# andrewcsmith/vox_box.rs

Hardware: AMD Instinct MI355X
Metric: frames/sec (pitch+LPC+formants), 48 kHz 25 ms/10 ms hop, 1→8 MI355X (higher is better)
Workload: dtype f64

## Files before the change

vox_box.rs_amd/csrc/vbx_device.hpp:

```cpp
#pragma once

#include <hip/hip_runtime.h>
#include <stdint.h>

#define VBX_WAVE 64

namespace vbx {


__device__ __forceinline__ double readlane_f64(double v, int lane) {
    int lo = __double2loint(v), hi = __double2hiint(v);
    lo = __builtin_amdgcn_readlane(lo, lane);
    hi = __builtin_amdgcn_readlane(hi, lane);
    return __hiloint2double(hi, lo);
}

__device__ __forceinline__ double readfirstlane_f64(double v) {
    int lo = __double2loint(v), hi = __double2hiint(v);
    lo = __builtin_amdgcn_readfirstlane(lo);
    hi = __builtin_amdgcn_readfirstlane(hi);
    return __hiloint2double(hi, lo);
}

template <int CTRL>
__device__ __forceinline__ double dpp_f64(double v) {
    int lo = __double2loint(v), hi = __double2hiint(v);
    lo = __builtin_amdgcn_update_dpp(0, lo, CTRL, 0xf, 0xf, true);
    hi = __builtin_amdgcn_update_dpp(0, hi, CTRL, 0xf, 0xf, true);
    return __hiloint2double(hi, lo);
}

constexpr int DPP_ROW_BCAST15 = 0x142, DPP_ROW_BCAST31 = 0x143;

constexpr int DPP_ROW_ROR1 = 0x121, DPP_ROW_ROR2 = 0x122, DPP_ROW_ROR4 = 0x124, DPP_ROW_ROR8 = 0x128;
constexpr int DPP_WAVE_SHL1 = 0x130;
constexpr int DPP_WAVE_SHR1 = 0x138;

__device__ __forceinline__ double from_next_lane(double v) { return dpp_f64<DPP_WAVE_SHL1>(v); }
__device__ __forceinline__ double from_prev_lane(double v) { return dpp_f64<DPP_WAVE_SHR1>(v); }

__device__ __forceinline__ double rounded(double v) { asm volatile("" : "+v"(v)); return v; }

__device__ __forceinline__ double wave_sum(double v) {
    v = rounded(v);
    v += dpp_f64<DPP_ROW_ROR8>(v);
    v += dpp_f64<DPP_ROW_ROR4>(v);
    v += dpp_f64<DPP_ROW_ROR2>(v);
    v += dpp_f64<DPP_ROW_ROR1>(v);
    double a = readlane_f64(v, 0), b = readlane_f64(v, 16), c = readlane_f64(v, 32), d = readlane_f64(v, 48);
    return (a + b) + (c + d);
}

template <int CTRL, int ROW_MASK>
__device__ __forceinline__ double dpp_f64_or_zero(double v) {
    int lo = __double2loint(v), hi = __double2hiint(v);
    lo = __builtin_amdgcn_update_dpp(0, lo, CTRL, ROW_MASK, 0xf, false);
    hi = __builtin_amdgcn_update_dpp(0, hi, CTRL, ROW_MASK, 0xf, false);
    return __hiloint2double(hi, lo);
}
__device__ __forceinline__ double wave_inclusive_scan(double v) {
    v += dpp_f64<0x111>(v);
    v += dpp_f64<0x112>(v);
    v += dpp_f64<0x114>(v);
    v += dpp_f64<0x118>(v);
    v += dpp_f64_or_zero<DPP_ROW_BCAST15, 0xA>(v);
    v += dpp_f64_or_zero<DPP_ROW_BCAST31, 0xC>(v);
    return v;
}

__device__ __forceinline__ double wave_max(double v) {
    v = fmax(v, dpp_f64<DPP_ROW_ROR8>(v));
    v = fmax(v, dpp_f64<DPP_ROW_ROR4>(v));
    v = fmax(v, dpp_f64<DPP_ROW_ROR2>(v));
    v = fmax(v, dpp_f64<DPP_ROW_ROR1>(v));
    double a = readlane_f64(v, 0), b = readlane_f64(v, 16), c = readlane_f64(v, 32), d = readlane_f64(v, 48);
    return fmax(fmax(a, b), fmax(c, d));
}

__device__ __forceinline__ double wave_sum_shfl(double v) {
    for (int o = 32; o > 0; o >>= 1) v += __shfl_xor(v, o, 64);
    return readfirstlane_f64(v);
}

__device__ __forceinline__ int lane_id() { return (int)(threadIdx.x & 63u); }

constexpr long XCD_RUN = 1024;
__device__ __forceinline__ long xcd_item(long b, long n) {
    constexpr long T = 8 * XCD_RUN;
    const long tile = b / T;
    if ((tile + 1) * T > n) return b;
    const long j = b - tile * T;
    return tile * T + (j & 7) * XCD_RUN + (j >> 3);
}

constexpr int DPP_QUAD_XOR1 = 0xB1;
constexpr int DPP_QUAD_REV = 0x1B;
constexpr int DPP_ROW_HALF_MIRROR = 0x141;
constexpr int DPP_ROW_MIRROR = 0x140;

template <int G>
__device__ __forceinline__ double group_sum(double v) {
    static_assert(G == 4 || G == 8 || G == 16 || G == 32 || G == 64, "group size");
    v = rounded(v);
    v += dpp_f64<DPP_QUAD_XOR1>(v);
    v += dpp_f64<DPP_QUAD_REV>(v);
    if (G >= 8) v += dpp_f64<DPP_ROW_HALF_MIRROR>(v);
    if (G >= 16) v += dpp_f64<DPP_ROW_MIRROR>(v);
    if (G == 64) {
        v += dpp_f64<DPP_ROW_BCAST15>(v);
        v += dpp_f64<DPP_ROW_BCAST31>(v);
        return readlane_f64(v, 63);
    }
    if (G == 32) {
        const double a = readlane_f64(v, 0), b = readlane_f64(v, 16), c = readlane_f64(v, 32), d = readlane_f64(v, 48);
        return (lane_id() < 32) ? (a + b) : (c + d);
    }
    return v;
}

__device__ __forceinline__ void wave_sync() {
    __builtin_amdgcn_fence(__ATOMIC_ACQ_REL, "wavefront");
    __builtin_amdgcn_wave_barrier();
}

__device__ __forceinline__ double rcp_nr1(double a) {
    double r = __builtin_amdgcn_rcp(a);
    return fma(fma(-a, r, 1.0), r, r);
}
__device__ __forceinline__ double rcp_nr2(double a) {
    double r = __builtin_amdgcn_rcp(a);
    r = fma(fma(-a, r, 1.0), r, r);
    return fma(fma(-a, r, 1.0), r, r);
}

__device__ __forceinline__ double div_exact_small(double x, double denom, double r) {
    const double q = x * r;
    const double rem = fma(-q, denom, x);
    return fma(rem, r, q);
}
__device__ __forceinline__ double pcm16_value(int s) { return div_exact_small((double)s, 32767.0, 1.0 / 32767.0); }


template <typename T> struct cx { T re, im; };
using c64 = cx<double>;
using c32 = cx<float>;

template <typename T> __device__ __forceinline__ cx<T> cmk(T re, T im) { cx<T> z; z.re = re; z.im = im; return z; }
template <typename T> __device__ __forceinline__ cx<T> cadd(cx<T> a, cx<T> b) { return cmk<T>(a.re + b.re, a.im + b.im); }
template <typename T> __device__ __forceinline__ cx<T> csub(cx<T> a, cx<T> b) { return cmk<T>(a.re - b.re, a.im - b.im); }
template <typename T> __device__ __forceinline__ cx<T> cneg(cx<T> a) { return cmk<T>(-a.re, -a.im); }
template <typename T> __device__ __forceinline__ cx<T> cmul(cx<T> a, cx<T> b) {
    return cmk<T>(a.re * b.re - a.im * b.im, a.re * b.im + a.im * b.re);
}
template <typename T> __device__ __forceinline__ cx<T> cmad(cx<T> a, cx<T> b, cx<T> c) {
    return cmk<T>(fma(a.re, b.re, fma(-a.im, b.im, c.re)), fma(a.re, b.im, fma(a.im, b.re, c.im)));
}
__device__ __forceinline__ double cdiv_recip(double ns) {
#ifdef VBX_IEEE_CDIV
    return 1.0 / ns;
#else
    return rcp_nr2(ns);
#endif
}
__device__ __forceinline__ float cdiv_recip(float ns) { return 1.0f / ns; }
template <typename T> __device__ __forceinline__ cx<T> cdiv(cx<T> a, cx<T> b) {
    T ns = b.re * b.re + b.im * b.im;
    T inv = cdiv_recip(ns);
    T re = a.re * b.re + a.im * b.im;
    T im = a.im * b.re - a.re * b.im;
    return cmk<T>(re * inv, im * inv);
}
template <typename T> __device__ __forceinline__ T cnorm(cx<T> a) { return hypot(a.re, a.im); }
template <typename T> __device__ __forceinline__ bool ciszero(cx<T> a) { return a.re == T(0) && a.im == T(0); }
template <typename T> __device__ __forceinline__ cx<T> csqrt(cx<T> z) {
    T r = hypot(z.re, z.im);
    if (r == T(0)) return cmk<T>(T(0), z.im);
    if (z.re >= T(0)) {
        T t = sqrt(T(0.5) * (r + z.re));
        return cmk<T>(t, z.im / (T(2) * t));
    }
    T t = sqrt(T(0.5) * (r - z.re));
    return cmk<T>(fabs(z.im) / (T(2) * t), copysign(t, z.im));
}

}
```

vox_box.rs_amd/csrc/vbx_pitch_refine.hpp:

```cpp
#pragma once
#include <type_traits>

#include "vbx_device.hpp"
#include "vbx_kernels.hpp"

namespace vbx {


__device__ __forceinline__ double fma_sc(double p, double x, const double c) {
    double r;
    asm("v_fma_f64 %0, %1, %2, %3" : "=v"(r) : "v"(p), "v"(x), "s"(c));
    return r;
}

__device__ __forceinline__ double sin_poly(double x) {
    const double x2 = x * x;
    double p = -1.9572941063391261231e-20;
    p = fma_sc(p, x2, 8.2206352466243297170e-18);
    p = fma_sc(p, x2, -2.8114572543455207632e-15);
    p = fma_sc(p, x2, 7.6471637318198164759e-13);
    p = fma_sc(p, x2, -1.6059043836821614599e-10);
    p = fma_sc(p, x2, 2.5052108385441718775e-08);
    p = fma_sc(p, x2, -2.7557319223985890653e-06);
    p = fma_sc(p, x2, 1.9841269841269841270e-04);
    p = fma_sc(p, x2, -8.3333333333333333333e-03);
    p = fma_sc(p, x2, 1.6666666666666666667e-01);
    return x * fma(-x2, p, 1.0);
}
__device__ __forceinline__ double cos_poly(double x) {
    const double x2 = x * x;
    double p = 8.8967913924505732867e-22;
    p = fma_sc(p, x2, -4.1103176233121648585e-19);
    p = fma_sc(p, x2, 1.5619206968586226462e-16);
    p = fma_sc(p, x2, -4.7794773323873852974e-14);
    p = fma_sc(p, x2, 1.1470745597729724714e-11);
    p = fma_sc(p, x2, -2.0876756987868098979e-09);
    p = fma_sc(p, x2, 2.7557319223985890653e-07);
    p = fma_sc(p, x2, -2.4801587301587301587e-05);
    p = fma_sc(p, x2, 1.3888888888888888889e-03);
    p = fma_sc(p, x2, -4.1666666666666666667e-02);
    p = fma(p, x2, 0.5);
    return fma(-x2, p, 1.0);
}

__device__ __forceinline__ double cos_0_pi(double theta) { return -sin_poly(theta - 1.57079632679489661923); }

__device__ __forceinline__ double y_at(const double *y, int nvalid, int idx) {
    return (idx < nvalid) ? y[idx] : 0.0;
}
__device__ __forceinline__ double y_at_padded(const double *y, int nvalid, int idx) {
    return y[(idx < nvalid) ? idx : nvalid - 1];
}


template <int G>
__device__ __forceinline__ double sinc_terms_general(const double *y, int nvalid, int ylen, int offset, int nl, int nr,
                                                     double phil, double phir, int max_depth, int lig = -1) {
    if (lig < 0) lig = lane_id() & (G - 1);
    const int side = lig & 1;
    const double ph = side ? phir : phil;
    const double s0 = sinpi(ph);
    const double inv_dd = 1.0 / (ph + (double)max_depth);
    const int ibase = side ? (offset + nl) : (offset + nr);
    double acc = 0.0;
    for (int n = (lig >> 1); n <= max_depth; n += G / 2) {
        const double a = M_PI * (ph + (double)n);
        int idx = side ? (ibase + n) : (ibase - n);
        idx = (idx < 0) ? 0 : idx;
        idx = (idx >= ylen) ? (ylen - 1) : idx;
        const double r_lag = y_at(y, nvalid, idx);
        const double sgn_s0 = (n & 1) ? -s0 : s0;
        const double first = sgn_s0 * rcp_nr2(a);
        const double second = fma(0.5, cos_0_pi(a * inv_dd), 0.5);
        acc = fma(r_lag * first, second, acc);
    }
    return acc;
}

struct sinc_stream_t {
    double pn, C, d, kappa, acc0, acc1;
    const double *yp;
};

template <int NSTEP>
__device__ __forceinline__ void sinc_stream_init(sinc_stream_t &s, const double *y, int side, int n0, int ibase_l, int ibase_r,
                                                 double phil, double phir, int max_depth) {
    constexpr double S = (double)NSTEP;
    const double ph = side ? phir : phil;
    const double h2 = M_PI * rcp_nr2(ph + (double)max_depth);
    s.pn = ph + (double)n0;
    const double theta0 = h2 * s.pn, delta = h2 * S;
    s.C = cos_0_pi(theta0);
    s.d = cos_0_pi(theta0 + delta) - s.C;
    const double sh = sin_poly(0.5 * delta);
    s.kappa = 4.0 * sh * sh;
    s.yp = y + (side ? (ibase_r + n0) : (ibase_l - n0));
    s.acc0 = 0.0; s.acc1 = 0.0;
}

template <int NSTEP>
__device__ __forceinline__ void sinc_stream_block4(sinc_stream_t &s, const int step) {
    constexpr double S = (double)NSTEP;
    const double y0 = s.yp[0], y1 = s.yp[step], y2 = s.yp[2 * step], y3 = s.yp[3 * step];
    const double p0 = s.pn, p1 = s.pn + S, p2 = s.pn + 2.0 * S, p3 = s.pn + 3.0 * S;
    const double q01 = p0 * p1, q23 = p2 * p3;
    const double r = rcp_nr1(q01 * q23);
    const double r01 = r * q23, r23 = r * q01;
    const double t0 = y0 * (r01 * p1), t1 = y1 * (r01 * p0), t2 = y2 * (r23 * p3), t3 = y3 * (r23 * p2);
    s.acc0 += t0; s.acc1 = fma(t0, s.C, s.acc1);
    s.C += s.d; s.d = fma(-s.kappa, s.C, s.d);
    s.acc0 += t1; s.acc1 = fma(t1, s.C, s.acc1);
    s.C += s.d; s.d = fma(-s.kappa, s.C, s.d);
    s.acc0 += t2; s.acc1 = fma(t2, s.C, s.acc1);
    s.C += s.d; s.d = fma(-s.kappa, s.C, s.d);
    s.acc0 += t3; s.acc1 = fma(t3, s.C, s.acc1);
    s.C += s.d; s.d = fma(-s.kappa, s.C, s.d);
    s.pn += 4.0 * S;
    s.yp += 4 * step;
}

template <int NSTEP>
__device__ __forceinline__ void sinc_stream_tail(sinc_stream_t &s, const int step, const int rem) {
    constexpr double S = (double)NSTEP;
    const double y0 = s.yp[0], y1 = (rem > 1) ? s.yp[step] : 0.0, y2 = (rem > 2) ? s.yp[2 * step] : 0.0;
    const double p0 = s.pn, p1 = s.pn + S, p2 = s.pn + 2.0 * S;
    const double q01 = p0 * p1;
    const double r = rcp_nr1(q01 * p2);
    const double r01 = r * p2;
    const double t0 = y0 * (r01 * p1), t1 = y1 * (r01 * p0), t2 = y2 * (r * q01);
    s.acc0 += t0; s.acc1 = fma(t0, s.C, s.acc1);
    s.C += s.d; s.d = fma(-s.kappa, s.C, s.d);
    s.acc0 += t1; s.acc1 = fma(t1, s.C, s.acc1);
    s.C += s.d;
    s.acc0 += t2; s.acc1 = fma(t2, s.C, s.acc1);
}

__device__ __forceinline__ double sinc_stream_result(const sinc_stream_t &s, int n0, double k) {
    const double acc = s.acc0 + s.acc1;
    return rounded(((n0 & 1) ? -acc : acc) * k);
}

template <int G>
__device__ __forceinline__ double sinc_terms_fast(const double *y, int ibase_l, int ibase_r,
                                                  double phil, double phir, int max_depth) {
    constexpr int NSTEP = G / 2;
    const int lig = lane_id() & (G - 1);
    const int side = lig & 1;
    const int n0 = lig >> 1;
    const double s0 = sin_poly(M_PI * fmin(phil, phir));
    const int nterms = (n0 <= max_depth) ? (max_depth - n0) / NSTEP + 1 : 0;
    sinc_stream_t s;
    sinc_stream_init<NSTEP>(s, y, side, n0, ibase_l, ibase_r, phil, phir, max_depth);
    const int step = side ? NSTEP : -NSTEP;
    int j = 0;
    for (; j + 4 <= nterms; j += 4) sinc_stream_block4<NSTEP>(s, step);
    if (j < nterms) sinc_stream_tail<NSTEP>(s, step, nterms - j);
    return sinc_stream_result(s, n0, s0 * (0.5 * 0.31830988618379067154));
}

__device__ __forceinline__ double sinc_terms_fast_cell(const double *yp0, int side, int n0, int nterms, double dmd,
                                                       double phil, double phir) {
    constexpr int NSTEP = 32;
    constexpr double S = (double)NSTEP;
    const int step = side ? NSTEP : -NSTEP;
    const double s0 = sin_poly(M_PI * fmin(phil, phir));
    sinc_stream_t s;
    const double ph = side ? phir : phil;
    const double h2 = M_PI * rcp_nr2(ph + dmd);
    s.pn = ph + (double)n0;
    const double theta0 = h2 * s.pn, delta = h2 * S;
    s.C = cos_0_pi(theta0);
    s.d = cos_0_pi(theta0 + delta) - s.C;
    const double sh = sin_poly(0.5 * delta);
    s.kappa = 4.0 * sh * sh;
    s.yp = yp0;
    s.acc0 = 0.0; s.acc1 = 0.0;
    int j = 0;
    for (; j + 4 <= nterms; j += 4) sinc_stream_block4<NSTEP>(s, step);
    if (j < nterms) sinc_stream_tail<NSTEP>(s, step, nterms - j);
    return sinc_stream_result(s, n0, s0 * (0.5 * 0.31830988618379067154));
}

template <int VG>
__device__ __forceinline__ double sinc_terms_fast_dual(const double *y, int ibase_l, int ibase_r,
                                                       double phil, double phir, int max_depth) {
    constexpr int NSTEP = VG / 2;
    const int n0 = lane_id() & (VG / 2 - 1);
    const double s0 = sin_poly(M_PI * fmin(phil, phir));
    const int nterms = (n0 <= max_depth) ? (max_depth - n0) / NSTEP + 1 : 0;
    sinc_stream_t sl, sr;
    sinc_stream_init<NSTEP>(sl, y, 0, n0, ibase_l, ibase_r, phil, phir, max_depth);
    sinc_stream_init<NSTEP>(sr, y, 1, n0, ibase_l, ibase_r, phil, phir, max_depth);
    int j = 0;
    for (; j + 4 <= nterms; j += 4) { sinc_stream_block4<NSTEP>(sl, -NSTEP); sinc_stream_block4<NSTEP>(sr, NSTEP); }
    if (j < nterms) { sinc_stream_tail<NSTEP>(sl, -NSTEP, nterms - j); sinc_stream_tail<NSTEP>(sr, NSTEP, nterms - j); }
    const double k = s0 * (0.5 * 0.31830988618379067154);
    return sinc_stream_result(sl, n0, k) + sinc_stream_result(sr, n0, k);
}

template <int G, bool DUAL = false>
__device__ __forceinline__ double sinc_interp(const double *y, int nvalid, int ylen, int offset, int nx,
                                              double x, int max_depth, bool active, int &st,
                                              unsigned *terms = nullptr, bool trusted = false) {
    bool summed = false, fast = false;
    double special = 0.0, phil = 0.5, phir = 0.5;
    int nl = 0, nr = 1;
    if (active && trusted) {
        const double fl = floor(x);
        nl = (int)fl;
        nr = nl + 1;
        phil = x - fl;
        phir = 1.0 - phil;
        if (fabs(x - (double)nl) < 1.0e-10) special = y[offset + nl];
        else if (fabs(x - (double)nr) < 1.0e-10) special = y[offset + nr];
        else {
            if ((offset + nr) < max_depth) max_depth = offset + nr;
            if ((offset + nl + max_depth) >= nx) max_depth = nx - offset + nl - 1;
            summed = true; fast = true;
        }
    } else if (active) {
        if (nx < 1) special = __builtin_nan("");
        else if (x > (double)nx) {
            const int idx = offset + nx - 1;
            if (idx < 0 || idx >= ylen) st |= 4; else special = y_at(y, nvalid, idx);
        } else if (x < 0.0) special = y_at(y, nvalid, 0);
        else {
            const double fl = floor(x);
            nl = (fl > 0.0) ? (int)fl : 0;
            nr = nl + 1;
            phil = x - (double)nl;
            phir = 1.0 - phil;
            if (fabs(x - (double)nl) < 1.0e-10) {
                const int idx = offset + nl;
                if (idx < 0 || idx >= ylen) st |= 4; else special = y_at(y, nvalid, idx);
            } else if (fabs(x - (double)nr) < 1.0e-10) {
                const int idx = offset + nr;
                if (idx < 0 || idx >= ylen) st |= 4; else special = y_at(y, nvalid, idx);
            } else {
                if ((offset + nr) < max_depth) max_depth = ((offset + nr) < 0) ? 0 : (offset + nr);
                if ((offset + nl + max_depth) >= nx) max_depth = nx - offset + nl - 1;
                if (max_depth < 0 || offset + nr >= ylen) st |= 4;
                else {
                    summed = true;
                    fast = !(x != x) && max_depth <= offset + nr && offset + nl >= 0 &&
                           offset + nl + max_depth < nvalid && offset + nr < nvalid;
                }
            }
        }
    }
    double acc = 0.0;
    if (terms != nullptr && summed) *terms += 2u * (unsigned)(max_depth + 1);
    if (summed) {
        if constexpr (DUAL) {
            if (fast) acc = sinc_terms_fast_dual<2 * G>(y, offset + nr, offset + nl, phil, phir, max_depth);
            else {
                const int p = lane_id() & (G - 1);
                acc = rounded(sinc_terms_general<2 * G>(y, nvalid, ylen, offset, nl, nr, phil, phir, max_depth, 2 * p)) +
                      rounded(sinc_terms_general<2 * G>(y, nvalid, ylen, offset, nl, nr, phil, phir, max_depth, 2 * p + 1));
            }
        } else {
            if (fast) acc = sinc_terms_fast<G>(y, offset + nr, offset + nl, phil, phir, max_depth);
            else acc = sinc_terms_general<G>(y, nvalid, ylen, offset, nl, nr, phil, phir, max_depth);
        }
    }
    const double total = group_sum<G>(acc);
    return summed ? total : special;
}

__device__ __forceinline__ bool sinc_bracket_trusted(double a0, double b0, int nvalid, int ylen, int offset, int nx, int depth) {
    if (!(a0 >= 0.0 && b0 <= (double)nx && b0 - a0 <= 2.5)) return false;
    const int lo = (int)floor(a0), hi = (int)floor(b0);
    bool ok = true;
    for (int nl = lo; nl <= hi; nl++) {
        const int nr = nl + 1;
        int D = depth;
        if ((offset + nr) < D) D = ((offset + nr) < 0) ? 0 : (offset + nr);
        if ((offset + nl + D) >= nx) D = nx - offset + nl - 1;
        ok = ok && D >= 0 && offset + nr < ylen && D <= offset + nr && offset + nl >= 0 && offset + nl + D < nvalid &&
             offset + nr < nvalid && offset + nr >= 1;
    }
    return ok;
}

template <int G>
__device__ __forceinline__ void improve_extremum_sinc(const double *y, int nvalid, int ylen, int offset, int nx,
                                                      double ixmid, int depth, bool active,
                                                      double &xmid, double &ymid, int &st,
                                                      unsigned *terms = nullptr, unsigned *evals = nullptr,
                                                      double bar = -__builtin_inf(), bool *pruned = nullptr,
                                                      bool negate = false ) {
#pragma clang fp contract(off)
    const double golden = 1. - 0.6180339887498948482045868343656381177203091798057628621;
    const double sqrt_epsilon = 1.4901161193847656e-08;
    const double eps = 2.220446049250313e-16;
    const double tol = 1e-10;
    xmid = 0.; ymid = 0.;
    bool run = active;
    if (active) {
        if (ixmid == 0.) { xmid = 0.; ymid = y_at(y, nvalid, 0); run = false; }
        else if (ixmid >= (double)nx) {
            run = false;
            if (nx < 1 || nx - 1 >= ylen) st |= 4;
            else { xmid = (double)nx; ymid = y_at(y, nvalid, nx - 1); }
        } else if (!(ixmid - 1. < ixmid + 1.)) { st |= 4; run = false; }
    }
    double a = ixmid - 1., b = ixmid + 1.;
    const bool trusted = run && sinc_bracket_trusted(a, b, nvalid, ylen, offset, nx, depth);
    double v = a + golden * (b - a);
    double fv = sinc_interp<G>(y, nvalid, ylen, offset, nx, v, depth, run, st, terms, trusted);
    if (negate) fv = -fv;
    if (evals != nullptr && run) *evals += 1u;
    double x = v, w = v, fx = fv, fw = fv;
    bool done = !run;
    const bool prunable = pruned != nullptr && run && a >= (double)(-offset);
    if (pruned != nullptr) {
        const double ub = (fv <= 1.) ? fv : 1.;
        *pruned = prunable && ub < bar;
        done = done || *pruned;
    }
    for (int it = 1; it <= 60; it++) {
        const double range = b - a;
        const double middle_range = (a + b) * 0.5;
        const double tol_act = sqrt_epsilon * fabs(x) + tol / 3.;
        if (!done && fabs(x - middle_range) + range * 0.5 <= 2. * tol_act) done = true;
        if (!__any(!done)) break;
        double new_step = (x < middle_range) ? golden * (b - x) : golden * (a - x);
        if (fabs(x - w) >= tol_act) {
            const double t = (x - w) * (fx - fv);
            double q = (x - v) * (fx - fw);
            double p = (x - v) * q - (x - w) * t;
            q = 2. * q - t;
            if (q > 0.) p = -p; else q = -q;
            if (fabs(p) < fabs(new_step * q) && p > q * (a - x + 2. * tol_act) && p < q * (b - x - 2. * tol_act))
                new_step = p / q;
        }
        if (fabs(new_step) < tol_act) new_step = (new_step > 0.) ? tol_act : -tol_act;
        const double t = x + new_step;
        double ft = sinc_interp<G>(y, nvalid, ylen, offset, nx, t, depth, !done, st, terms, trusted);
        if (negate) ft = -ft;
        if (evals != nullptr && !done) *evals += 1u;
        if (!done) {
            if (ft <= fx) {
                if (t < x) b = x; else a = x;
                v = w; w = x; x = t;
                fv = fw; fw = fx; fx = ft;
            } else {
                if (t < x) a = t; else b = t;
                if (ft <= fw || fabs(w - x) < eps) {
                    v = w; w = t;
                    fv = fw; fw = ft;
                } else if (ft <= fv || fabs(v - x) < eps || fabs(v - w) < eps) {
                    v = t;
                    fv = ft;
                }
            }
            if (prunable && fx < bar) { *pruned = true; done = true; }
        }
    }
    if (run) { xmid = x; ymid = fx; }
}

__device__ __forceinline__ bool improve_extremum_sinc_wave(const double *y, int nvalid, int ylen, int offset, int nx,
                                                           double ixmid, int depth, double &xmid, double &ymid,
                                                           unsigned &terms, unsigned &evals, double bar, bool &pruned) {
#pragma clang fp contract(off)
    const double golden = 1. - 0.6180339887498948482045868343656381177203091798057628621;
    const double sqrt_epsilon = 1.4901161193847656e-08;
    const double eps = 2.220446049250313e-16;
    const double tol = 1e-10;
    if (__any(ixmid == 0. || ixmid >= (double)nx || !(ixmid - 1. < ixmid + 1.))) return false;
    double a = ixmid - 1., b = ixmid + 1.;
    if (!__any(sinc_bracket_trusted(a, b, nvalid, ylen, offset, nx, depth))) return false;
    const int lane = lane_id();
    const int side = lane & 1, n0 = lane >> 1;
    struct cell_t { int nl, nterms; unsigned tinc; double dmd; const double *yp0; };
    cell_t ca{-0x7fffffff, 0, 0u, 0.0, y}, cb{-0x7fffffff, 0, 0u, 0.0, y};
    bool a_is_older = true;
    auto fill = [&](cell_t &c, int nl) {
        c.nl = nl;
        const int nr = nl + 1;
        int md = depth;
        if ((offset + nr) < md) md = offset + nr;
        if ((offset + nl + md) >= nx) md = nx - offset + nl - 1;
        c.tinc = 2u * (unsigned)(md + 1);
        c.dmd = (double)md;
        c.nterms = (n0 <= md) ? (md - n0) / 32 + 1 : 0;
        c.yp0 = y + (side ? (offset + nl + n0) : (offset + nr - n0));
    };
    auto eval = [&](double x) -> double {
        const double fl = floor(x);
        const int nl = (int)fl;
        const double phil = x - fl, phir = 1.0 - phil;
        if (__any(phil < 1.0e-10)) return y[offset + nl];
        if (__any(phir < 1.0e-10)) return y[offset + nl + 1];
        if (__any(nl == ca.nl)) {
            a_is_older = false;
            terms += ca.tinc;
            return group_sum<64>(sinc_terms_fast_cell(ca.yp0, side, n0, ca.nterms, ca.dmd, phil, phir));
        }
        if (__any(nl != cb.nl)) {
            if (a_is_older) { fill(ca, nl); a_is_older = false; terms += ca.tinc;
                              return group_sum<64>(sinc_terms_fast_cell(ca.yp0, side, n0, ca.nterms, ca.dmd, phil, phir)); }
            fill(cb, nl);
        }
        a_is_older = true;
        terms += cb.tinc;
        return group_sum<64>(sinc_terms_fast_cell(cb.yp0, side, n0, cb.nterms, cb.dmd, phil, phir));
    };
    double v = a + golden * (b - a);
    double fv = eval(v);
    evals += 1u;
    double x = v, w = v, fx = fv, fw = fv;
    const bool prunable = __any(a >= (double)(-offset));
    pruned = false;
    if (prunable && __any(((fv <= 1.) ? fv : 1.) < bar)) { pruned = true; return true; }
    for (int it = 1; it <= 60; it++) {
        const double range = b - a;
        const double middle_range = (a + b) * 0.5;
        const double tol_act = sqrt_epsilon * fabs(x) + tol / 3.;
        if (__any(fabs(x - middle_range) + range * 0.5 <= 2. * tol_act)) break;
        double new_step = __any(x < middle_range) ? golden * (b - x) : golden * (a - x);
        if (__any(fabs(x - w) >= tol_act)) {
            const double t = (x - w) * (fx - fv);
            double q = (x - v) * (fx - fw);
            double p = (x - v) * q - (x - w) * t;
            q = 2. * q - t;
            if (__any(q > 0.)) p = -p; else q = -q;
            if (__any(fabs(p) < fabs(new_step * q) && p > q * (a - x + 2. * tol_act) && p < q * (b - x - 2. * tol_act))) {
                asm volatile("" ::: "memory");
                new_step = p / q;
            }
        }
        if (__any(fabs(new_step) < tol_act)) new_step = __any(new_step > 0.) ? tol_act : -tol_act;
        const double t = x + new_step;
        const double ft = eval(t);
        evals += 1u;
        if (__any(ft <= fx)) {
            if (__any(t < x)) b = x; else a = x;
            v = w; w = x; x = t;
            fv = fw; fw = fx; fx = ft;
        } else {
            if (__any(t < x)) a = t; else b = t;
            if (__any(ft <= fw || fabs(w - x) < eps)) {
                v = w; w = t;
                fv = fw; fw = ft;
            } else if (__any(ft <= fv || fabs(v - x) < eps || fabs(v - w) < eps)) {
                v = t;
                fv = ft;
            }
        }
        if (prunable && __any(fx < bar)) { pruned = true; return true; }
    }
    xmid = x; ymid = fx;
    return true;
}

constexpr int Y_PAD = 16;
#ifndef VBX_EXP_PB
#define VBX_EXP_PB 5
#endif
constexpr int PB = VBX_EXP_PB;
__device__ __forceinline__ double block_abs_sum(const double *yp) {
    double s = fabs(yp[0]) + fabs(yp[1]);
#pragma unroll
    for (int i = 2; i + 1 < PB; i += 2) s += fabs(yp[i]) + fabs(yp[i + 1]);
    if (PB & 1) s += fabs(yp[PB - 1]);
    return s;
}
typedef unsigned short cand_t;
constexpr int PG = 16;
constexpr int PNG = 64 / PG;
constexpr int GROUP_PATH_MIN_CAND = 32;
#ifndef VBX_EXP_RG
#define VBX_EXP_RG 16
#endif
#ifndef VBX_EXP_GROUP_KMAX
#define VBX_EXP_GROUP_KMAX 4
#endif
constexpr int RG = VBX_EXP_RG;
#ifndef VBX_EXP_DUAL_MIN_CAND
#define VBX_EXP_DUAL_MIN_CAND 6
#endif
constexpr int DUAL_MIN_CAND = VBX_EXP_DUAL_MIN_CAND;

__device__ __forceinline__ void cand_from_peak(const double *ys, int kk, double sample_rate, int offset,
                                               double &freq, double &nn, const bool f32 = false) {
    const double peak = ys[kk], peak_rev = ys[kk - 1], peak_fwd = ys[kk + 1];
    if (f32) {
#pragma clang fp contract(off)
        const double dr = 0.5 * (double)(float)(peak_fwd - peak_rev);
        const double d2r = 2. * peak - (double)(float)(peak_rev - peak_fwd);
        freq = (double)(float)(sample_rate / (double)(float)((double)kk + dr / d2r));
        nn = (double)(float)((double)(float)(sample_rate / freq) - (double)offset);
        return;
    }
    const double dr = 0.5 * (peak_fwd - peak_rev);
    const double d2r = 2. * peak - (peak_rev - peak_fwd);
    freq = sample_rate / ((double)kk + dr / d2r);
    nn = sample_rate / freq - (double)offset;
}

constexpr int BOUND_HEAD = 8;

__device__ __forceinline__ double taper_upper(double theta) {
    const double t = theta * theta;
    double p = fma(t, 2.48015873015873016e-05, -1.38888888888888894e-03);
    p = fma(p, t, 4.16666666666666644e-02);
    p = fma(p, t, -0.5);
    return fma(0.5, fma(p, t, 1.0), 0.5) * (1.0 + 1.0e-15);
}

__device__ __forceinline__ void abs_range_idx(int nblk, int i0, int i1, int &j0, int &j1) {
    i0 = (i0 < 0) ? 0 : i0;
    const int last = PB * nblk - 1;
    i1 = (i1 > last) ? last : i1;
    const bool empty = i1 < i0;
    j0 = empty ? 0 : (int)((unsigned)i0 / PB);
    j1 = empty ? 0 : (int)((unsigned)i1 / PB) + 1;
}
template <int STEP, int TB>
__device__ __forceinline__ double first_eval_tail(const double *p16, int nblk, int offset, int nl, int nr, int D, int lo0,
                                                  double phil, double phir, double hl, double hr) {
    double tail = 0.0;
    for (int lo = lo0; lo <= D;) {
        double sl[TB], sr[TB];
#pragma unroll
        for (int q = 0, l = lo; q < TB; q++, l *= STEP) {
            const int hi = (2 * l < D + 1) ? 2 * l : D + 1;
            int a0 = 0, a1 = 0, b0 = 0, b1 = 0;
            if (l <= D) {
                abs_range_idx(nblk, offset + nr - (hi - 1), offset + nr - l, a0, a1);
                abs_range_idx(nblk, offset + nl + l, offset + nl + hi - 1, b0, b1);
            }
            sl[q] = p16[a1] - p16[a0];
            sr[q] = p16[b1] - p16[b0];
        }
#pragma unroll
        for (int q = 0; q < TB; q++) {
            if (lo > D) break;
            const double pl = phil + (double)lo, pr = phir + (double)lo;
            const double cl = rcp_nr1(pl) * taper_upper(hl * pl);
            const double cr = rcp_nr1(pr) * taper_upper(hr * pr);
            tail = fma(cl, sl[q], tail);
            tail = fma(cr, sr[q], tail);
            lo *= STEP;
        }
    }
    return tail;
}

__device__ __forceinline__ double first_eval_bound(const double *ys, const double *p16, int nblk, int nvalid, int ylen,
                                                   int offset, int nx, double nn, int depth) {
    const double INF = __builtin_inf();
    if (nn == 0. || nn >= (double)nx || !(nn - 1. < nn + 1.)) return INF;
    double v0;
    {
#pragma clang fp contract(off)
        const double golden = 1. - 0.6180339887498948482045868343656381177203091798057628621;
        const double ba = nn - 1., bb = nn + 1.;
        if (!(ba >= (double)(-offset))) return INF;
        v0 = ba + golden * (bb - ba);
    }
    if (nx < 1 || v0 > (double)nx || v0 < 0.0) return INF;
    const double fl = floor(v0);
    const int nl = (int)fl, nr = nl + 1;
    const double phil = v0 - (double)nl, phir = 1.0 - phil;
    if (fabs(v0 - (double)nl) < 1.0e-10 || fabs(v0 - (double)nr) < 1.0e-10) return INF;
    int D = depth;
    if ((offset + nr) < D) D = ((offset + nr) < 0) ? 0 : (offset + nr);
    if ((offset + nl + D) >= nx) D = nx - offset + nl - 1;
    if (D < 0 || offset + nr >= ylen || D > offset + nr || offset + nl < 0 || offset + nl + D >= ylen) return INF;
    const double s0 = sin_poly(M_PI * fmin(phil, phir)) * 0.31830988618379067154;
    const double hl = M_PI * rcp_nr1(phil + (double)D), hr = M_PI * rcp_nr1(phir + (double)D);
    double head = 0.0;
    const int nh = (BOUND_HEAD < D + 1) ? BOUND_HEAD : D + 1;
    {
        double cl = cos_0_pi(hl * phil), cr = cos_0_pi(hr * phir);
        double dl = cos_0_pi(hl * (phil + 1.0)) - cl, dr = cos_0_pi(hr * (phir + 1.0)) - cr;
        const double sl = sin_poly(0.5 * hl), sr = sin_poly(0.5 * hr);
        const double kl = 4.0 * sl * sl, kr = 4.0 * sr * sr;
        double yl[BOUND_HEAD], yr[BOUND_HEAD];
#pragma unroll
        for (int m = 0; m < BOUND_HEAD; m++) {
            const bool in = m < nh;
            yl[m] = y_at_padded(ys, nvalid, in ? offset + nr - m : 0);
            yr[m] = y_at_padded(ys, nvalid, in ? offset + nl + m : 0);
        }
#pragma unroll
        for (int m = 0; m < BOUND_HEAD; m++) {
            if (m >= nh) break;
            const double pl = phil + (double)m, pr = phir + (double)m;
            const double tl = yl[m] * rcp_nr1(pl) * fma(0.5, cl, 0.5);
            const double tr = yr[m] * rcp_nr1(pr) * fma(0.5, cr, 0.5);
            const double t = tl + tr;
            head += (m & 1) ? -t : t;
            cl += dl; dl = fma(-kl, cl, dl);
            cr += dr; dr = fma(-kr, cr, dr);
        }
    }
    head *= s0;
    double tail = first_eval_tail<2, 4>(p16, nblk, offset, nl, nr, D, nh, phil, phir, hl, hr);
    tail *= s0;
    const double ub = head + tail * (1.0 + 1.0e-9) + (1.0e-9 + 1.0e-11 * p16[nblk]);
    return (ub != ub) ? INF : ub;
}

__device__ __forceinline__ double first_eval_bound_quad(const double *ys, const double *p16, int nblk, int nvalid, int ylen,
                                                        int offset, int nx, double nn, int depth, int sub, bool have) {
    const double INF = __builtin_inf();
    bool inf = !have;
    double v0 = 0.;
    if (!inf) {
        if (nn == 0. || nn >= (double)nx || !(nn - 1. < nn + 1.)) inf = true;
        else {
#pragma clang fp contract(off)
            const double golden = 1. - 0.6180339887498948482045868343656381177203091798057628621;
            const double ba = nn - 1., bb = nn + 1.;
            if (!(ba >= (double)(-offset))) inf = true;
            v0 = ba + golden * (bb - ba);
        }
    }
    if (!inf && (nx < 1 || v0 > (double)nx || v0 < 0.0)) inf = true;
    int nl = 0, nr = 1, D = 0;
    double phil = 0.5, phir = 0.5;
    if (!inf) {
        const double fl = floor(v0);
        nl = (int)fl; nr = nl + 1;
        phil = v0 - (double)nl; phir = 1.0 - phil;
        if (fabs(v0 - (double)nl) < 1.0e-10 || fabs(v0 - (double)nr) < 1.0e-10) inf = true;
        D = depth;
        if ((offset + nr) < D) D = ((offset + nr) < 0) ? 0 : (offset + nr);
        if ((offset + nl + D) >= nx) D = nx - offset + nl - 1;
        if (D < 0 || offset + nr >= ylen || D > offset + nr || offset + nl < 0 || offset + nl + D >= ylen) inf = true;
    }
    double head = 0.0, tail = 0.0;
    if (!inf) {
        const double s0 = sin_poly(M_PI * fmin(phil, phir)) * 0.31830988618379067154;
        const double hl = M_PI * rcp_nr1(phil + (double)D), hr = M_PI * rcp_nr1(phir + (double)D);
        const int nh = (BOUND_HEAD < D + 1) ? BOUND_HEAD : D + 1;
        double yl[BOUND_HEAD / 4], yr[BOUND_HEAD / 4];
#pragma unroll
        for (int j = 0; j < BOUND_HEAD / 4; j++) {
            const int m = sub + 4 * j;
            const bool in = m < nh;
            yl[j] = y_at_padded(ys, nvalid, in ? offset + nr - m : 0);
            yr[j] = y_at_padded(ys, nvalid, in ? offset + nl + m : 0);
        }
#pragma unroll
        for (int j = 0; j < BOUND_HEAD / 4; j++) {
            const int m = sub + 4 * j;
            if (m >= nh) break;
            const double pl = phil + (double)m, pr = phir + (double)m;
            const double tl = yl[j] * rcp_nr1(pl) * fma(0.5, cos_0_pi(hl * pl), 0.5);
            const double tr = yr[j] * rcp_nr1(pr) * fma(0.5, cos_0_pi(hr * pr), 0.5);
            const double t = tl + tr;
            head += (m & 1) ? -t : t;
        }
        head *= s0;
        tail = first_eval_tail<16, 2>(p16, nblk, offset, nl, nr, D, nh << sub, phil, phir, hl, hr);
        tail *= s0;
    }
    head = group_sum<4>(head);
    tail = group_sum<4>(tail);
    const double ub = head + tail * (1.0 + 1.0e-9) + (1.0e-9 + 1.0e-11 * p16[nblk]);
    return (inf || ub != ub) ? INF : ub;
}

__device__ __forceinline__ int pick_best(float *keys, int ncand, double bar, int lane) {
    double bv = -__builtin_inf(); int bi = 0x7fffffff;
    for (int i = lane; i < ncand; i += 64) { const double v = (double)keys[i]; if (v > bv) { bv = v; bi = i; } }
    const double gm = wave_max(bv);
    int pick = (bv == gm) ? bi : 0x7fffffff;
    for (int o = 32; o > 0; o >>= 1) { const int other = __shfl_xor(pick, o, 64); pick = (other < pick) ? other : pick; }
    if (pick == 0x7fffffff || !(gm >= bar)) return -1;
    if (lane == 0) keys[pick] = -__builtin_inff();
    wave_sync();
    return pick;
}


__device__ __forceinline__ int pick_best_pred(float *keys, const cand_t *cand_list, const double *ys, int ncand, double bar, int lane) {
    double bv = -__builtin_inf(); int bi = 0x7fffffff;
    for (int i = lane; i < ncand; i += 64) {
        const float kv = keys[i];
        if (kv > -__builtin_inff() && (double)kv >= bar) {
            const int k = (int)cand_list[i];
            double p = fmin(ys[k - 1], ys[k + 1]);
            if (!(p == p)) p = __builtin_inf();
            if (bi == 0x7fffffff || p > bv) { bv = p; bi = i; }
        }
    }
    const double gm = wave_max(bv);
    int pick = (bi != 0x7fffffff && bv == gm) ? bi : 0x7fffffff;
    for (int o = 32; o > 0; o >>= 1) { const int other = __shfl_xor(pick, o, 64); pick = (other < pick) ? other : pick; }
    if (pick == 0x7fffffff) return -1;
    if (lane == 0) keys[pick] = -__builtin_inff();
    wave_sync();
    return pick;
}


__host__ __device__ constexpr int pitch_refine_lds_bytes(int n, int nst = 0, int cap = 0) {
    const int m = (nst > 0) ? nst : n;
    return (m + Y_PAD + ((((m + PB - 1) / PB) + 2) & ~1)) * 8 + ((cap > 0) ? cap : n / 4 + 8) * (int)(sizeof(float) + sizeof(cand_t));
}

inline int pitch_curve_reach(int n, double sample_rate, double fmin) {
    if (!(fmin > 0.0) || !(sample_rate > 0.0)) return 0;
    const double reach = 2.0 * ceil(sample_rate / fmin) + 16.0;
    if (!(reach < (double)n)) return 0;
    return ((int)reach + 1) & ~1;
}
inline int pitch_curve_entries(int n, double sample_rate, double fmin) {
    if ((n & 1) || !(fmin > 0.0) || !(sample_rate > 0.0)) return 0;
    const double reach = 2.0 * ceil(sample_rate / fmin) + 16.0;
    if (!(reach < (double)n)) return 0;
    int m = (int)reach;
    if (m < n / 2 + 2) m = n / 2 + 2;
    m = (m + 1) & ~1;
    return (m < n) ? m : 0;
}

struct pitch_params_t { double sample_rate, threshold, fmin, fmax; int kmax; int full_off; int f32 = 0; int ncurve = 0; };
__host__ __device__ constexpr int pitch_full_list_entries(int n) { return n / 4 + 2; }

template <int STAGE = 0>
__device__ __forceinline__ bool pitch_refine_store(double *ys, int n, const pitch_params_t &pp, long f,
                                                   double *__restrict__ out_cand, long cand_ld,
                                                   int32_t *__restrict__ out_count, int32_t *__restrict__ status,
                                                   unsigned long long *__restrict__ work, double unc_tol = 0.0,
                                                   double2 *full = nullptr, int *io_ncand = nullptr, int cand_cap = 0,
                                                   uint16_t *list_at = nullptr) {
    const int lane = lane_id();
    const double sample_rate = pp.sample_rate, threshold = pp.threshold, fmin = pp.fmin, fmax = pp.fmax;
    const int kmax = pp.kmax;
    const bool f32 = pp.f32 != 0;
    const int nst = (pp.ncurve > 0) ? pp.ncurve : n;
    const int nblk = (nst + PB - 1) / PB;
    double *p16 = ys + nst + Y_PAD;
    float *keys = reinterpret_cast<float *>(p16 + ((nblk + 2) & ~1));
    cand_t *cand_list = (STAGE == 1 && list_at != nullptr) ? reinterpret_cast<cand_t *>(list_at)
                                                           : reinterpret_cast<cand_t *>(keys + ((STAGE == 2 && cand_cap > 0) ? cand_cap : n / 4 + 8));
    const int b = (int)floor(0.5 * (double)n);
    const int offset = -b - 1;
    const int nx = b - offset;
    const int ylen = 2 * n;
    const int nvalid = nst + Y_PAD;

    VBX_PHASE_INIT();
    int ncand = 0;
    if constexpr (STAGE == 2) ncand = *io_ncand;
    else {
    int npeak = 0;
    bool unsure = false;
    for (int base = 0; base < b; base += 64) {
        const int k = base + lane;
        bool peak = false;
        if (k >= 1 && k + 1 < b) {
            const double c = ys[k];
            const double d1 = c - ys[k - 1], d2 = c - ys[k + 1];
            peak = (ys[k - 1] < c) && (ys[k + 1] < c);
            unsure = unsure || (fabs((d1 < d2) ? d1 : d2) <= unc_tol);
        }
        const unsigned long long mask = __ballot(peak);
        if (peak) cand_list[npeak + __popcll(mask & ((1ull << lane) - 1ull))] = (cand_t)k;
        npeak += __popcll(mask);
    }
    wave_sync();
    if (unc_tol > 0.0 && __any(unsure)) return false;
    VBX_PHASE(work, f, 6);
    unsure = false;
    for (int base = 0; base < npeak; base += 64) {
        const int i = base + lane;
        bool pass = false;
        int k = 0;
        if (i < npeak) {
            k = cand_list[i];
            double freq, nn;
            cand_from_peak(ys, k, sample_rate, offset, freq, nn, f32);
            pass = (freq == 0.0) || (freq > fmin && freq < fmax);
            if (unc_tol > 0.0) {
                const double c = ys[k], d2r = 2. * c - (ys[k - 1] - ys[k + 1]), dr = 0.5 * (ys[k + 1] - ys[k - 1]);
                const double dlag = unc_tol * (1.0 + 4.0 * fabs(dr / d2r)) / fabs(d2r);
                const double tol_f = 2.0 * freq * dlag / fabs((double)k + dr / d2r);
                if (!(fabs(freq - fmin) > tol_f && fabs(freq - fmax) > tol_f)) unsure = true;
            }
        }
        wave_sync();
        const unsigned long long mask = __ballot(pass);
        if (pass) cand_list[ncand + __popcll(mask & ((1ull << lane) - 1ull))] = (cand_t)k;
        ncand += __popcll(mask);
        wave_sync();
    }

    if (unc_tol > 0.0 && __any(unsure)) return false;
    VBX_PHASE(work, f, 7);
    }
    if constexpr (STAGE == 1) { *io_ncand = ncand; return true; }

    const bool in_order = full != nullptr || kmax > ncand || f32;
    if (!in_order) {
        const int per = (nblk + 63) >> 6;
        double tot = 0.0;
        for (int q = 0; q < per; q++) {
            const int j = lane * per + q;
            if (j < nblk) tot += block_abs_sum(ys + PB * j);
        }
        const double incl = wave_inclusive_scan(tot);
        double run = incl - tot;
        if (lane == 0) p16[0] = 0.0;
        for (int q = 0; q < per; q++) {
            const int j = lane * per + q;
            if (j < nblk) {
                run += block_abs_sum(ys + PB * j);
                p16[j + 1] = run;
            }
        }
        wave_sync();
        const bool quad = ((ncand + 15) / 16) * 7 < ((ncand + 63) / 64) * 25;
        if (quad) {
            for (int base = 0; base < ncand; base += 16) {
                const int c = base + (lane >> 2);
                const bool have = c < ncand;
                double freq = 0., nn = 0.;
                if (have) cand_from_peak(ys, cand_list[c], sample_rate, offset, freq, nn, f32);
                const double ub = first_eval_bound_quad(ys, p16, nblk, nvalid, ylen, offset, nx, nn, 1200, lane & 3, have);
                const double kb = (ub <= 1.) ? ub : ((ub != ub) ? __builtin_inf() : ((ub == __builtin_inf()) ? ub : 1.));
                if (have && (lane & 3) == 0) keys[c] = __double2float_ru(kb);
            }
        } else {
            for (int c = lane; c < ncand; c += 64) {
                double freq, nn;
                cand_from_peak(ys, cand_list[c], sample_rate, offset, freq, nn, f32);
                const double ub = first_eval_bound(ys, p16, nblk, nvalid, ylen, offset, nx, nn, 1200);
                const double kb = (ub <= 1.) ? ub : ((ub != ub) ? __builtin_inf() : ((ub == __builtin_inf()) ? ub : 1.));
                keys[c] = __double2float_ru(kb);
            }
        }
        wave_sync();
    }

    VBX_PHASE(work, f, 8);
    int st = 0;
    int kept = 0;
    double lf = 0.0, ls = 0.0;
    bool any_nan = false;
    int li = 0;
    { lf = 0.0; ls = threshold; li = ncand; kept = 1; }
    const bool fullm = full != nullptr;
    if (fullm && lane == 0) full[ncand] = double2{0.0, threshold};

#define VBX_BAR() ((!fullm && !f32 && kept == kmax) ? readlane_f64(ls, kmax - 1) : -__builtin_inf())
    auto insert = [&](double f_g, double s_g, int c_g) {
        if (s_g != s_g) any_nan = true;
        if (fullm) { if (lane == 0) full[c_g] = double2{f_g, s_g}; return; }
        const int pos = __popcll(__ballot(lane < kept && (ls > s_g || (ls == s_g && li < c_g))));
        const double pf = from_prev_lane(lf), ps = from_prev_lane(ls);
        const int pi = __builtin_amdgcn_update_dpp(0, li, DPP_WAVE_SHR1, 0xf, 0xf, true);
        if (lane > pos) { lf = pf; ls = ps; li = pi; }
        if (lane == pos) { lf = f_g; ls = s_g; li = c_g; }
        kept = (kept + 1 < kmax) ? kept + 1 : kmax;
    };
    unsigned cterms = 0, cevals = 0;

    int next_full = ncand - 1;
    unsigned nterms = 0, nevals = 0;
    int group_lanes = RG;
    if (ncand <= GROUP_PATH_MIN_CAND && !(kmax >= VBX_EXP_GROUP_KMAX && ncand >= 4)) {
        for (;;) {
            const double bar = VBX_BAR();
            const int c = in_order ? next_full-- : pick_best_pred(keys, cand_list, ys, ncand, bar, lane);
            if (c < 0) break;
            double freq, nn, xmid, ymid;
            cand_from_peak(ys, cand_list[c], sample_rate, offset, freq, nn, f32);
            bool dropped = false;
#ifndef VBX_EXP_NO_WAVE_BRENT
            if (!improve_extremum_sinc_wave(ys, nvalid, ylen, offset, nx, nn, 1200, xmid, ymid, cterms, cevals, bar, dropped))
#endif
                improve_extremum_sinc<64>(ys, nvalid, ylen, offset, nx, nn, 1200, true, xmid, ymid, st, &cterms, &cevals, bar, &dropped);
            if (dropped) continue;
            double xm, ym;
            {
#pragma clang fp contract(off)
                xm = xmid + (double)offset;
                ym = ymid;
                if (ym > 1.) ym = 1. / ym;
                xm = sample_rate / (f32 ? (double)(float)xm : xm);
                if (f32) { xm = (double)(float)xm; ym = (double)(float)ym; }
            }
            insert(xm, ym, c);
        }
    } else {
      auto run_groups = [&](auto pg_tag, auto dual_tag) {
        constexpr int PG = decltype(pg_tag)::value;
        constexpr bool DUAL = decltype(dual_tag)::value;
        bool exhausted = false;
        const int gid = lane / PG;
        int ci = -1, it = 0;
        bool special = false, safe = false, trusted = false;
        double ba = 0., bb = 0., v = 0., w = 0., x = 0., fv = 0., fw = 0., fx = 0., xmid = 0., ymid = 0.;
        constexpr unsigned long long LEADERS = (PG == 16) ? 0x0001000100010001ull : (PG == 8) ? 0x0101010101010101ull
                                             : (PG == 32) ? 0x0000000100000001ull : (PG == 4) ? 0x1111111111111111ull : 1ull;
        const double golden = 1. - 0.6180339887498948482045868343656381177203091798057628621;
        const double sqrt_epsilon = 1.4901161193847656e-08, eps = 2.220446049250313e-16, tol = 1e-10;
        for (;;) {
#pragma clang fp contract(off)
            bool finished = false;
            double range = 0., middle_range = 0., tol_act = 0.;
            if (ci >= 0) {
                if (special) finished = true;
                else if (it > 0) {
                    range = bb - ba;
                    middle_range = (ba + bb) * 0.5;
                    tol_act = sqrt_epsilon * fabs(x) + tol / 3.;
                    if (it > 60 || fabs(x - middle_range) + range * 0.5 <= 2. * tol_act) { finished = true; xmid = x; ymid = fx; }
                }
            }
            if (__any(finished)) {
                unsigned long long fm = __ballot(finished) & LEADERS;
                double xm = xmid + (double)offset;
                double ym = ymid;
                if (ym > 1.) ym = 1. / ym;
                double cf = sample_rate / (f32 ? (double)(float)xm : xm), cs = ym;
                if (f32) { cf = (double)(float)cf; cs = (double)(float)cs; }
                while (fm) {
                    const int ld = __builtin_ctzll(fm);
                    fm &= fm - 1;
                    insert(readlane_f64(cf, ld), readlane_f64(cs, ld), __builtin_amdgcn_readlane(ci, ld));
                }
                if (finished) ci = -1;
            }
            {
                unsigned long long im = __ballot(ci < 0) & LEADERS;
                while (im != 0ull && !exhausted) {
                    const int c = in_order ? next_full-- : pick_best_pred(keys, cand_list, ys, ncand, VBX_BAR(), lane);
                    if (c < 0) { exhausted = true; break; }
                    const int g = __builtin_ctzll(im) / PG;
                    im &= im - 1ull;
                    if (gid == g) {
                        ci = c;
                        double freq, nn;
                        cand_from_peak(ys, cand_list[ci], sample_rate, offset, freq, nn, f32);
                        it = 0; special = false; xmid = 0.; ymid = 0.;
                        if (nn == 0.) { special = true; xmid = 0.; ymid = ys[0]; }
                        else if (nn >= (double)nx) { special = true; xmid = (double)nx; ymid = y_at(ys, nvalid, nx - 1); }
                        else if (!(nn - 1. < nn + 1.)) { special = true; st |= 4; }
                        ba = nn - 1.; bb = nn + 1.;
                        safe = ba >= (double)(-offset);
                        trusted = !special && sinc_bracket_trusted(ba, bb, nvalid, ylen, offset, nx, 1200);
                    }
                }
            }
            if (!__any(ci >= 0)) break;
            const double bar = VBX_BAR();

            bool need = false;
            double t = 0.;
            if (ci >= 0 && !special) {
                if (it == 0) { v = ba + golden * (bb - ba); t = v; }
                else {
                    double new_step = (x < middle_range) ? golden * (bb - x) : golden * (ba - x);
                    if (fabs(x - w) >= tol_act) {
                        const double tt = (x - w) * (fx - fv);
                        double q = (x - v) * (fx - fw);
                        double pp = (x - v) * q - (x - w) * tt;
                        q = 2. * q - tt;
                        if (q > 0.) pp = -pp; else q = -q;
                        if (fabs(pp) < fabs(new_step * q) && pp > q * (ba - x + 2. * tol_act) && pp < q * (bb - x - 2. * tol_act))
                            new_step = pp / q;
                    }
                    if (fabs(new_step) < tol_act) new_step = (new_step > 0.) ? tol_act : -tol_act;
                    t = x + new_step;
                }
                need = true;
            }
            const double ft = sinc_interp<PG, DUAL>(ys, nvalid, ylen, offset, nx, t, 1200, need, st, &nterms, trusted);
            nevals += need ? 1u : 0u;
            if (need) {
                if (it == 0) {
                    x = v; w = v; fv = ft; fx = ft; fw = ft; it = 1;
                    const double ub = (ft <= 1.) ? ft : 1.;
                    if (ub < bar && safe) ci = -1;
                } else {
                    if (ft <= fx) {
                        if (t < x) bb = x; else ba = x;
                        v = w; w = x; x = t;
                        fv = fw; fw = fx; fx = ft;
                    } else {
                        if (t < x) ba = t; else bb = t;
                        if (ft <= fw || fabs(w - x) < eps) {
                            v = w; w = t;
                            fv = fw; fw = ft;
                        } else if (ft <= fv || fabs(v - x) < eps || fabs(v - w) < eps) {
                            v = t;
                            fv = ft;
                        }
                    }
                    it++;
                    if (safe && fx < bar) ci = -1;
                }
            }
        }
      };
      const bool dual_ok = in_order || (kmax >= 8 && ncand >= 12);
      if (RG == 16 && dual_ok && ncand >= DUAL_MIN_CAND) { run_groups(std::integral_constant<int, RG / 2>{}, std::true_type{}); group_lanes = RG / 2; }
      else run_groups(std::integral_constant<int, RG>{}, std::false_type{});
    }
#undef VBX_BAR
    VBX_PHASE(work, f, 9);
    const int total_cand = ncand + 1;
    st = __any(st & 4) ? 4 : 0;
    if (total_cand > 1 && (any_nan || threshold != threshold)) st |= 8;
    int code = 0;
    if (st & 4) code = 4; else if (st & 8) code = 3;
    if (fullm) {
        wave_sync();
        if (pp.full_off < 0) {
            __builtin_amdgcn_fence(__ATOMIC_RELEASE, "agent");
            __builtin_amdgcn_fence(__ATOMIC_ACQUIRE, "agent");
            double2 *lds_list = reinterpret_cast<double2 *>(ys);
            for (int i = lane; i < total_cand; i += 64) lds_list[i] = full[i];
            full = lds_list;
            wave_sync();
        }
        double *row = out_cand + f * cand_ld;
        const int total = (code == 0) ? total_cand : 0;
        for (int i0 = 0; i0 < total; i0 += 64) {
            const int i = i0 + lane;
            const double2 me = (i < total) ? full[i] : double2{0.0, 0.0};
            int rank = 0;
            for (int j = 0; j < total; j++) {
                const double sj = full[j].y;
                rank += (sj > me.y || (sj == me.y && j < i)) ? 1 : 0;
            }
            if (i < total && rank < kmax) *reinterpret_cast<double2 *>(row + 2 * rank) = me;
        }
        for (int i = total + lane; i < kmax; i += 64) *reinterpret_cast<double2 *>(row + 2 * i) = double2{0.0, 0.0};
    } else if (lane < kmax) {
        const bool valid = (code == 0) && lane < kept;
        double2 o;
        o.x = valid ? lf : 0.0;
        o.y = valid ? ls : 0.0;
        *reinterpret_cast<double2 *>(out_cand + f * cand_ld + 2 * lane) = o;
    }
    if (lane == 0) {
        if (out_count != nullptr) out_count[f] = (code == 0) ? total_cand : 0;
        if (status != nullptr) status[f] = code;
    }
    if (work != nullptr) {
        const bool leader = (lane & (group_lanes - 1)) == 0;
        unsigned long long te = leader ? nterms : 0u, ev = leader ? nevals : 0u;
        for (int o = 32; o > 0; o >>= 1) { te += __shfl_xor(te, o, 64); ev += __shfl_xor(ev, o, 64); }
        if (lane == 0) {
            unsigned long long *w = work + 4 * (f & (PITCH_WORK_SLOTS - 1));
            atomicAdd(w + 0, 1ull); atomicAdd(w + 1, (unsigned long long)ncand);
            atomicAdd(w + 2, ev + cevals); atomicAdd(w + 3, te + cterms);
        }
    }
    return true;
}

}
```

Before: 37.76 million.

## Scalarize Brent sinc refinement state and fuse trig setup into one polynomial pass

The Brent-minimiser interpolation eval now keeps its bracket, abscissa and cell index wave-uniform via readfirstlane, so the compiler can hold them in scalar registers. The two-entry cell cache is simplified to a swap. The inlined sinc-term setup computes cos through shifted sin polynomials and packs the two sin evaluations into one polynomial call with DPP lane merging. Counter updates are deferred to the end. It also precomputes the block count and applies the sign via a bit flip, cutting VALU work and divergence bookkeeping, at some risk of subtle numerical differences in the trig path.

```diff
diff --git a/vox_box.rs_amd/csrc/vbx_device.hpp b/vox_box.rs_amd/csrc/vbx_device.hpp
--- a/vox_box.rs_amd/csrc/vbx_device.hpp
+++ b/vox_box.rs_amd/csrc/vbx_device.hpp
@@ -27,6 +27,14 @@
     int lo = __double2loint(v), hi = __double2hiint(v);
     lo = __builtin_amdgcn_update_dpp(0, lo, CTRL, 0xf, 0xf, true);
     hi = __builtin_amdgcn_update_dpp(0, hi, CTRL, 0xf, 0xf, true);
+    return __hiloint2double(hi, lo);
+}
+
+template <int CTRL, int ROW_MASK, int BANK_MASK>
+__device__ __forceinline__ double dpp_f64_into(double old, double v) {
+    int lo = __double2loint(v), hi = __double2hiint(v);
+    lo = __builtin_amdgcn_update_dpp(__double2loint(old), lo, CTRL, ROW_MASK, BANK_MASK, false);
+    hi = __builtin_amdgcn_update_dpp(__double2hiint(old), hi, CTRL, ROW_MASK, BANK_MASK, false);
     return __hiloint2double(hi, lo);
 }
 
@@ -93,6 +101,8 @@
     return tile * T + (j & 7) * XCD_RUN + (j >> 3);
 }
 
+constexpr int DPP_QUAD_IDENTITY = 0xE4;
+constexpr int DPP_ROW_SHR4 = 0x114;
 constexpr int DPP_QUAD_XOR1 = 0xB1;
 constexpr int DPP_QUAD_REV = 0x1B;
 constexpr int DPP_ROW_HALF_MIRROR = 0x141;
diff --git a/vox_box.rs_amd/csrc/vbx_pitch_refine.hpp b/vox_box.rs_amd/csrc/vbx_pitch_refine.hpp
--- a/vox_box.rs_amd/csrc/vbx_pitch_refine.hpp
+++ b/vox_box.rs_amd/csrc/vbx_pitch_refine.hpp
@@ -13,7 +13,7 @@
     return r;
 }
 
-__device__ __forceinline__ double sin_poly(double x) {
+__device__ __forceinline__ double sin_poly_q(double x) {
     const double x2 = x * x;
     double p = -1.9572941063391261231e-20;
     p = fma_sc(p, x2, 8.2206352466243297170e-18);
@@ -25,8 +25,9 @@
     p = fma_sc(p, x2, 1.9841269841269841270e-04);
     p = fma_sc(p, x2, -8.3333333333333333333e-03);
     p = fma_sc(p, x2, 1.6666666666666666667e-01);
-    return x * fma(-x2, p, 1.0);
-}
+    return fma(-x2, p, 1.0);
+}
+__device__ __forceinline__ double sin_poly(double x) { return x * sin_poly_q(x); }
 __device__ __forceinline__ double cos_poly(double x) {
     const double x2 = x * x;
     double p = 8.8967913924505732867e-22;
@@ -152,29 +153,6 @@
     sinc_stream_t s;
     sinc_stream_init<NSTEP>(s, y, side, n0, ibase_l, ibase_r, phil, phir, max_depth);
     const int step = side ? NSTEP : -NSTEP;
-    int j = 0;
-    for (; j + 4 <= nterms; j += 4) sinc_stream_block4<NSTEP>(s, step);
-    if (j < nterms) sinc_stream_tail<NSTEP>(s, step, nterms - j);
-    return sinc_stream_result(s, n0, s0 * (0.5 * 0.31830988618379067154));
-}
-
-__device__ __forceinline__ double sinc_terms_fast_cell(const double *yp0, int side, int n0, int nterms, double dmd,
-                                                       double phil, double phir) {
-    constexpr int NSTEP = 32;
-    constexpr double S = (double)NSTEP;
-    const int step = side ? NSTEP : -NSTEP;
-    const double s0 = sin_poly(M_PI * fmin(phil, phir));
-    sinc_stream_t s;
-    const double ph = side ? phir : phil;
-    const double h2 = M_PI * rcp_nr2(ph + dmd);
-    s.pn = ph + (double)n0;
-    const double theta0 = h2 * s.pn, delta = h2 * S;
-    s.C = cos_0_pi(theta0);
-    s.d = cos_0_pi(theta0 + delta) - s.C;
-    const double sh = sin_poly(0.5 * delta);
-    s.kappa = 4.0 * sh * sh;
-    s.yp = yp0;
-    s.acc0 = 0.0; s.acc1 = 0.0;
     int j = 0;
     for (; j + 4 <= nterms; j += 4) sinc_stream_block4<NSTEP>(s, step);
     if (j < nterms) sinc_stream_tail<NSTEP>(s, step, nterms - j);
@@ -369,13 +347,13 @@
     const double eps = 2.220446049250313e-16;
     const double tol = 1e-10;
     if (__any(ixmid == 0. || ixmid >= (double)nx || !(ixmid - 1. < ixmid + 1.))) return false;
-    double a = ixmid - 1., b = ixmid + 1.;
+    double a = readfirstlane_f64(ixmid - 1.), b = readfirstlane_f64(ixmid + 1.);
     if (!__any(sinc_bracket_trusted(a, b, nvalid, ylen, offset, nx, depth))) return false;
     const int lane = lane_id();
     const int side = lane & 1, n0 = lane >> 1;
-    struct cell_t { int nl, nterms; unsigned tinc; double dmd; const double *yp0; };
-    cell_t ca{-0x7fffffff, 0, 0u, 0.0, y}, cb{-0x7fffffff, 0, 0u, 0.0, y};
-    bool a_is_older = true;
+    const int sign_bit = (n0 & 1) << 31;
+    struct cell_t { int nl, nblk; unsigned tinc; double dmd; int nterms; const double *yp0; };
+    cell_t cur{-0x7fffffff, 0, 0u, 0.0, 0, y}, oth{-0x7fffffff, 0, 0u, 0.0, 0, y};
     auto fill = [&](cell_t &c, int nl) {
         c.nl = nl;
         const int nr = nl + 1;
@@ -385,35 +363,58 @@
         c.tinc = 2u * (unsigned)(md + 1);
         c.dmd = (double)md;
         c.nterms = (n0 <= md) ? (md - n0) / 32 + 1 : 0;
+        c.nblk = ((31 <= md) ? (md - 31) / 32 + 1 : 0) >> 2;
         c.yp0 = y + (side ? (offset + nl + n0) : (offset + nr - n0));
     };
+    unsigned nterms_s = 0u, nevals_s = 1u;
     auto eval = [&](double x) -> double {
         const double fl = floor(x);
-        const int nl = (int)fl;
+        int nlv = (int)fl;
+        asm("" : "+v"(nlv));
+        const int nl = __builtin_amdgcn_readfirstlane(nlv);
         const double phil = x - fl, phir = 1.0 - phil;
-        if (__any(phil < 1.0e-10)) return y[offset + nl];
-        if (__any(phir < 1.0e-10)) return y[offset + nl + 1];
-        if (__any(nl == ca.nl)) {
-            a_is_older = false;
-            terms += ca.tinc;
-            return group_sum<64>(sinc_terms_fast_cell(ca.yp0, side, n0, ca.nterms, ca.dmd, phil, phir));
-        }
-        if (__any(nl != cb.nl)) {
-            if (a_is_older) { fill(ca, nl); a_is_older = false; terms += ca.tinc;
-                              return group_sum<64>(sinc_terms_fast_cell(ca.yp0, side, n0, ca.nterms, ca.dmd, phil, phir)); }
-            fill(cb, nl);
-        }
-        a_is_older = true;
-        terms += cb.tinc;
-        return group_sum<64>(sinc_terms_fast_cell(cb.yp0, side, n0, cb.nterms, cb.dmd, phil, phir));
+        if (__any(phil < 1.0e-10)) return readfirstlane_f64(y[offset + nl]);
+        if (__any(phir < 1.0e-10)) return readfirstlane_f64(y[offset + nl + 1]);
+        if (nl != cur.nl) {
+            if (nl != oth.nl) fill(oth, nl);
+            const cell_t t = cur; cur = oth; oth = t;
+        }
+        nterms_s += cur.tinc;
+        constexpr int NSTEP = 32;
+        constexpr double S = (double)NSTEP;
+        const int step = side ? NSTEP : -NSTEP;
+        sinc_stream_t s;
+        const double ph = side ? phir : phil;
+        const double h2 = M_PI * rcp_nr2(ph + cur.dmd);
+        s.pn = ph + (double)n0;
+        const double delta = h2 * S;
+        const double xc = fma(s.pn, h2, -1.57079632679489661923);
+        s.C = -(xc * sin_poly_q(xc));
+        const double xd = fma(s.pn, h2, delta) - 1.57079632679489661923;
+        s.d = fma(xd, -sin_poly_q(xd), -s.C);
+        double pmin;
+        asm("v_min_f64 %0, %1, %2" : "=v"(pmin) : "v"(phil), "v"(phir));
+        const double xs = dpp_f64_into<DPP_QUAD_IDENTITY, 0x8, 0x8>(0.5 * delta, M_PI * pmin);
+        const double sn = xs * sin_poly_q(xs);
+        const double k = readlane_f64(sn * (0.5 * 0.31830988618379067154), 63);
+        const double sh = dpp_f64_into<DPP_ROW_SHR4, 0x8, 0x8>(sn, sn);
+        s.kappa = 4.0 * sh * sh;
+        s.yp = cur.yp0;
+        s.acc0 = 0.0; s.acc1 = 0.0;
+        for (int j = 0; j < cur.nblk; j++) sinc_stream_block4<NSTEP>(s, step);
+        const int rest = cur.nterms - 4 * cur.nblk;
+        if (rest >= 4) sinc_stream_block4<NSTEP>(s, step);
+        if (rest & 3) sinc_stream_tail<NSTEP>(s, step, rest & 3);
+        const double acc = s.acc0 + s.acc1;
+        const double signed_acc = __hiloint2double(__double2hiint(acc) ^ sign_bit, __double2loint(acc));
+        return group_sum<64>(signed_acc * k);
     };
-    double v = a + golden * (b - a);
+    double v = readfirstlane_f64(a + golden * (b - a));
     double fv = eval(v);
-    evals += 1u;
     double x = v, w = v, fx = fv, fw = fv;
     const bool prunable = __any(a >= (double)(-offset));
     pruned = false;
-    if (prunable && __any(((fv <= 1.) ? fv : 1.) < bar)) { pruned = true; return true; }
+    if (prunable && __any(((fv <= 1.) ? fv : 1.) < bar)) { pruned = true; terms += nterms_s; evals += nevals_s; return true; }
     for (int it = 1; it <= 60; it++) {
         const double range = b - a;
         const double middle_range = (a + b) * 0.5;
@@ -426,21 +427,21 @@
             double p = (x - v) * q - (x - w) * t;
             q = 2. * q - t;
             if (__any(q > 0.)) p = -p; else q = -q;
-            if (__any(fabs(p) < fabs(new_step * q) && p > q * (a - x + 2. * tol_act) && p < q * (b - x - 2. * tol_act))) {
+            if (__any((int)(fabs(p) < fabs(new_step * q)) & (int)(p > q * (a - x + 2. * tol_act)) & (int)(p < q * (b - x - 2. * tol_act)))) {
                 asm volatile("" ::: "memory");
                 new_step = p / q;
             }
         }
         if (__any(fabs(new_step) < tol_act)) new_step = __any(new_step > 0.) ? tol_act : -tol_act;
-        const double t = x + new_step;
+        const double t = readfirstlane_f64(x + new_step);
         const double ft = eval(t);
-        evals += 1u;
+        nevals_s += 1u;
         if (__any(ft <= fx)) {
-            if (__any(t < x)) b = x; else a = x;
+            if (__any(t < x)) { asm volatile(""); b = x; } else { asm volatile(""); a = x; }
             v = w; w = x; x = t;
             fv = fw; fw = fx; fx = ft;
         } else {
-            if (__any(t < x)) a = t; else b = t;
+            if (__any(t < x)) { asm volatile(""); a = t; } else { asm volatile(""); b = t; }
             if (__any(ft <= fw || fabs(w - x) < eps)) {
                 v = w; w = t;
                 fv = fw; fw = ft;
@@ -449,9 +450,10 @@
                 fv = ft;
             }
         }
-        if (prunable && __any(fx < bar)) { pruned = true; return true; }
-    }
-    xmid = x; ymid = fx;
+        if (prunable && __any(fx < bar)) { pruned = true; break; }
+    }
+    terms += nterms_s; evals += nevals_s;
+    if (!pruned) { xmid = x; ymid = fx; }
     return true;
 }
 
```

Result: faster. 38.75 million (median of 6 runs) (+2.6%).
